# MaxChen228/pingpong-selfplay-ai

Measured on AMD Instinct MI355X. Metric: env-steps/sec (whole node) at 65536 arenas, 1/2/4/8 GPUs; CPU-ref baseline, higher is better.
Workload: dtype f64 env state / f32 QNet; 1 GPU; configs[2]: 65536 arenas/GPU, full DQN train_iterative loop (act both players + env tick + PER push/sample + double-DQN update + Adam + target sync); arenas_per_gpu=65536, global_arenas=65536, pool=8, batch=256, updates_per_vector_step=1, memory_size=1000000, parallelism=dp1 (arena shards, 1 all-reduce/update)

## Files before the change

### pingpong-selfplay-ai_amd/csrc/pm_dev.h

```cpp
#pragma once
#include <hip/hip_runtime.h>
#include <stdint.h>

#include "pongmi.h"

#ifdef PM_DIAG
static __device__ unsigned long long pm_diag_buf[256];
#define PM_STAMP(slot)                                                                 \
    do {                                                                               \
        if (threadIdx.x == 0 && blockIdx.x == 0) pm_diag_buf[(slot)] = __builtin_amdgcn_s_memrealtime(); \
    } while (0)
#define PM_STAMP_ANY(slot)                                                             \
    do {                                                                               \
        if (threadIdx.x == 0) pm_diag_buf[(slot)] = __builtin_amdgcn_s_memrealtime();  \
    } while (0)
static __device__ unsigned long long pm_diag_blk[8][4096];
#define PM_BLK_END()                                                                              \
    do {                                                                                          \
        __syncthreads();                                                                          \
        PM_BLK(2);                                                                                \
        if (threadIdx.x == 0 && blockIdx.x < 4096)                                                \
            pm_diag_blk[3][blockIdx.x] =                                                          \
                (unsigned long long)__smid() | ((unsigned long long)(__builtin_amdgcn_s_getreg(20 | (3 << 11)) & 15) << 16); \
    } while (0)
// ... 106 lines not shown
};

__device__ __forceinline__ U4 philox(uint32_t c0, uint32_t c1, uint32_t c2, uint32_t c3, uint64_t key) {
    uint32_t k0 = (uint32_t)key, k1 = (uint32_t)(key >> 32);
#pragma unroll
    for (int r = 0; r < 10; ++r) {
        const uint64_t p0 = (uint64_t)c0 * 0xD2511F53u, p1 = (uint64_t)c2 * 0xCD9E8D57u;
        const uint32_t hi0 = (uint32_t)(p0 >> 32), lo0 = (uint32_t)p0;
        const uint32_t hi1 = (uint32_t)(p1 >> 32), lo1 = (uint32_t)p1;
        const uint32_t n0 = hi1 ^ c1 ^ k0, n2 = hi0 ^ c3 ^ k1;
        c0 = n0; c1 = lo1; c2 = n2; c3 = lo0;
        k0 += 0x9E3779B9u; k1 += 0xBB67AE85u;
    }
    return {c0, c1, c2, c3};
}

__device__ __forceinline__ U4 philox64(uint32_t index, uint32_t tag, uint64_t ctr, uint64_t key) {
    return philox(index, tag, (uint32_t)ctr, (uint32_t)(ctr >> 32), key);
}

__device__ __forceinline__ double u53(uint32_t hi, uint32_t lo) {
    const uint64_t v = (((uint64_t)hi << 32) | lo) >> 11;
    return (double)v * 0x1.0p-53;
}
__device__ __forceinline__ int32_t below(uint32_t r, uint32_t n) {
    return (int32_t)(((uint64_t)r * n) >> 32);
}
__device__ __forceinline__ double det_ln_u1(uint32_t k) {
    int e = 31 - __builtin_clz(k);
    double m = (double)k / (double)(1u << e);
    if (m > 1.4142135623730951) { m = m * 0.5; e = e + 1; }
    const double s = (m - 1.0) / (m + 1.0), s2 = s * s;
    const double p = s2 * (0.66666666666666663 + s2 * (0.40000000000000002 + s2 * (0.28571428571428570 +
                     s2 * (0.22222222222222221 + s2 * (0.18181818181818182 + s2 * (0.15384615384615385 +
                     s2 * (0.13333333333333333 + s2 * (0.11764705882352941 + s2 * (0.10526315789473684 +
                     s2 * 0.09523809523809523)))))))));
    return (double)(e - 24) * 0.69314718055994531 + (2.0 * s + s * p);
}
__device__ __forceinline__ double det_cos_turn(double t) {
    const double q = floor(4.0 * t + 0.5);
    const double th = 6.2831853071795862 * (t - 0.25 * q);
    const double z = th * th;
    const double c = 1.0 + z * (-0.5 + z * (0.041666666666666664 + z * (-0.0013888888888888889 +
                     z * (2.4801587301587302e-05 + z * (-2.755731922398589e-07 + z * (2.0876756987868100e-09 +
                     z * -1.1470745597729725e-11))))));
    const double s = th * (1.0 + z * (-0.16666666666666666 + z * (0.0083333333333333332 + z * (-0.00019841269841269841 +
                     z * (2.7557319223985893e-06 + z * (-2.5052108385441720e-08 + z * (1.6059043836821613e-10 +
                     z * -7.6471637318198164e-13)))))));
    const int qi = (int)q & 3;
    return qi == 0 ? c : (qi == 1 ? -s : (qi == 2 ? -c : s));
}
__device__ __forceinline__ float normal(uint32_t a, uint32_t b) {
    const double r = sqrt(-2.0 * det_ln_u1((a >> 8) + 1u));
    return (float)(r * det_cos_turn((double)(b >> 8) * 0x1.0p-24));
}
__device__ __forceinline__ float scale_noise(float x) {
    const float s = x > 0.f ? 1.f : (x < 0.f ? -1.f : 0.f);
    return s * (float)sqrt((double)fabsf(x));
}

struct Arena {
    double x, y, vx, vy, spin, top, bot;
    int32_t sA, sB, bounces;
};

__device__ __forceinline__ Arena load_arena(const pm_env_state& s, int i) {
    Arena a;
    a.x = s.x[i]; a.y = s.y[i]; a.vx = s.vx[i]; a.vy = s.vy[i];
    a.spin = s.spin[i]; a.top = s.top[i]; a.bot = s.bot[i];
    a.sA = s.scoreA[i]; a.sB = s.scoreB[i]; a.bounces = s.bounces[i];
    return a;
}

template <bool WT, typename T>
__device__ __forceinline__ void st_out(T* p, T v) {
    if constexpr (WT) __hip_atomic_store(p, v, __ATOMIC_RELAXED, __HIP_MEMORY_SCOPE_AGENT);
    else *p = v;
}
typedef float pm_f4v __attribute__((ext_vector_type(4)));
template <bool WT>
__device__ __forceinline__ void st_f4(float4* p, float4 v) {
    if constexpr (WT) {
        const pm_f4v x = {v.x, v.y, v.z, v.w};
        asm volatile("global_store_dwordx4 %0, %1, off sc1" ::"v"(p), "v"(x) : "memory");
    } else {
        *p = v;
    }
}

template <bool WT = false>
__device__ __forceinline__ void store_arena(const pm_env_state& s, int i, const Arena& a) {
    st_out<WT>(&s.x[i], a.x); st_out<WT>(&s.y[i], a.y); st_out<WT>(&s.vx[i], a.vx); st_out<WT>(&s.vy[i], a.vy);
    st_out<WT>(&s.spin[i], a.spin); st_out<WT>(&s.top[i], a.top); st_out<WT>(&s.bot[i], a.bot);
    st_out<WT>(&s.scoreA[i], a.sA); st_out<WT>(&s.scoreB[i], a.sB); st_out<WT>(&s.bounces[i], a.bounces);
}

__device__ __forceinline__ void observe(const Arena& a, float* oA, float* oB) {
    oA[0] = (float)a.x; oA[1] = (float)(1.0 - a.y); oA[2] = (float)a.vx; oA[3] = (float)(-a.vy);
    oA[4] = (float)a.top; oA[5] = (float)a.bot; oA[6] = (float)a.spin;
    oB[0] = (float)a.x; oB[1] = (float)a.y; oB[2] = (float)a.vx; oB[3] = (float)a.vy;
    oB[4] = (float)a.bot; oB[5] = (float)a.top; oB[6] = (float)a.spin;
}

constexpr int kRowBlock = 256;

template <bool WT = false>
__device__ __forceinline__ void copy_rows7(float* __restrict__ dst, const float (*lds)[7], int i0, int n) {
    const int t = threadIdx.x;
    const int rows = min(kRowBlock, n - i0);
    float* base = dst + (size_t)i0 * 7;
    const float* src = &lds[0][0];
    if (rows == kRowBlock && (((uintptr_t)base) & 15) == 0) {
        float4* d4 = reinterpret_cast<float4*>(base);
        const float4* s4 = reinterpret_cast<const float4*>(__builtin_assume_aligned(src, 16));
#pragma unroll
        for (int f = t; f < kRowBlock * 7 / 4; f += kRowBlock) st_f4<WT>(d4 + f, s4[f]);
    } else {
        for (int f = t; f < rows * 7; f += kRowBlock) base[f] = src[f];
    }
}

__device__ __forceinline__ void store_rows7(float* __restrict__ dst, float (*lds)[7], const float* row, int i0,
                                            int n) {
    const int t = threadIdx.x;
#pragma unroll
    for (int k = 0; k < 7; ++k) lds[t][k] = row[k];
    __syncthreads();
    copy_rows7(dst, lds, i0, n);
    __syncthreads();
}

typedef float pm_f4u __attribute__((ext_vector_type(4), aligned(4)));
typedef float pm_f3u __attribute__((ext_vector_type(3), aligned(4)));
__device__ __forceinline__ void store_row7(float* __restrict__ dst, const float* v) {
    *reinterpret_cast<pm_f4u*>(dst) = pm_f4u{v[0], v[1], v[2], v[3]};
    *reinterpret_cast<pm_f3u*>(dst + 4) = pm_f3u{v[4], v[5], v[6]};
}

__device__ __forceinline__ void serve(Arena& a, double vx, double vy, double spin) {
    a.sA = 0; a.sB = 0; a.bounces = 0;
    a.top = 0.5; a.bot = 0.5; a.x = 0.5; a.y = 0.5;
    a.vx = vx; a.vy = vy; a.spin = spin;
}

__device__ __forceinline__ void sincos_serve(double x, double& s, double& c) {
    const double pio4 = 7.85398163397448278999e-01;
    const double pio2_1 = 1.57079632673412561417e+00, pio2_1t = 6.07710050650619224932e-11;
    const int n = x > pio4 ? 1 : (x < -pio4 ? -1 : 0);
    const double z0 = n > 0 ? x - pio2_1 : x + pio2_1;
    const double t = n > 0 ? pio2_1t : -pio2_1t;
    double y0 = z0 - t;
    double y1 = (z0 - y0) - t;
    y0 = n == 0 ? x : y0;
    y1 = n == 0 ? 0.0 : y1;
    const double S1 = -1.66666666666666324348e-01, S2 = 8.33333333332248946124e-03,
                 S3 = -1.98412698298579493134e-04, S4 = 2.75573137070700676789e-06,
                 S5 = -2.50507602534068634195e-08, S6 = 1.58969099521155010221e-10;
    const double z = y0 * y0, v = z * y0;
    const double rs = S2 + z * (S3 + z * (S4 + z * (S5 + z * S6)));
    const double ks = y0 - ((z * (0.5 * y1 - v * rs) - y1) - v * S1);
    const double C1 = 4.16666666666666019037e-02, C2 = -1.38888888888741095749e-03,
                 C3 = 2.48015872894767294178e-05, C4 = -2.75573143513906633035e-07,
                 C5 = 2.08757232129817482790e-09, C6 = -1.13596475577881948265e-11;
    const double rc = z * (C1 + z * (C2 + z * (C3 + z * (C4 + z * (C5 + z * C6)))));
    const double hz = 0.5 * z, w = 1.0 - hz;
    const double kc = w + (((1.0 - w) - hz) + (z * rc - y0 * y1));
    s = n == 0 ? ks : (n > 0 ? kc : -kc);
    c = n == 0 ? kc : (n > 0 ? -ks : ks);
}
// ... 168 lines not shown
```

### pingpong-selfplay-ai_amd/csrc/pm_per.h

```cpp
#pragma once
#include <hip/hip_runtime.h>
#include <stdint.h>

#include "pongmi.h"
#include "pm_dev.h"

namespace pm {

constexpr int PER_SUB = 64;
constexpr int PER_FAN = 16;
constexpr int PER_CHUNK = PER_SUB * PER_FAN;

__host__ __device__ inline int64_t per_pad(int64_t n_doubles) { return ((n_doubles * 8 + 255) / 256) * 256; }

struct PerTree {
    double* chunk;
    double* sub;
    float* leaf;
    int64_t nchunk, nsub;
};

__host__ __device__ inline PerTree per_tree(void* work, int64_t cap) {
    PerTree t;
    t.nsub = (cap + PER_SUB - 1) / PER_SUB;
    t.nchunk = (cap + PER_CHUNK - 1) / PER_CHUNK;
    char* w = reinterpret_cast<char*>(work);
    t.chunk = reinterpret_cast<double*>(w);
    t.sub = reinterpret_cast<double*>(w + per_pad(t.nchunk));
    t.leaf = reinterpret_cast<float*>(w + per_pad(t.nchunk) + per_pad(t.nsub));
    return t;
}

inline int64_t per_work_bytes(int64_t cap) {
    return per_pad((cap + PER_CHUNK - 1) / PER_CHUNK) + per_pad((cap + PER_SUB - 1) / PER_SUB) +
           ((cap * 4 + 255) / 256) * 256;
}

struct PushRange {
    int64_t pos, n, cap;
    float pval;
    __device__ __forceinline__ int64_t dist(int64_t e) const {
        const int64_t d = e - pos;
        return d < 0 ? d + cap : d;
    }
    __device__ __forceinline__ bool covers(int64_t e) const { return dist(e) < n; }
};

__device__ __forceinline__ double wave_incl_scan(double v, int lane) {
#pragma unroll
    for (int o = 1; o < 64; o <<= 1) {
        const double u = __shfl_up(v, o);
        if (lane >= o) v += u;
    }
    return v;
}

struct RingNodes {
    int64_t a0, na, nb;
    __device__ __forceinline__ int64_t count() const { return na + nb; }
    __device__ __forceinline__ int64_t at(int64_t k) const { return k < na ? a0 + k : k - na; }
};
__device__ __forceinline__ RingNodes ring_nodes(const PushRange& pr, int64_t g) {
    RingNodes r{pr.pos / g, 0, 0};
    if (pr.n <= 0) return r;
    const int64_t end1 = pr.pos + pr.n < pr.cap ? pr.pos + pr.n : pr.cap;
    r.na = (end1 - 1) / g - r.a0 + 1;
    const int64_t end2 = pr.pos + pr.n - pr.cap;
    r.nb = end2 > 0 ? (end2 - 1) / g + 1 : 0;
    return r;
}

__device__ __forceinline__ float prio_pow(float p, float alpha) {
    if (!(p > 0.f)) return 0.f;
    int e;
    double m = 2.0 * frexp((double)p, &e);
    e = e - 1;
    if (m > 1.4142135623730951) { m = m * 0.5; e = e + 1; }
    const double s = (m - 1.0) / (m + 1.0), s2 = s * s;
    const double q = s2 * (0.66666666666666663 + s2 * (0.40000000000000002 + s2 * (0.28571428571428570 +
                     s2 * (0.22222222222222221 + s2 * (0.18181818181818182 + s2 * (0.15384615384615385 +
                     s2 * (0.13333333333333333 + s2 * (0.11764705882352941 + s2 * (0.10526315789473684 +
                     s2 * 0.09523809523809523)))))))));
    const double y = (double)alpha * ((double)e * 0.69314718055994531 + (2.0 * s + s * q));
    const double k = floor(y * 1.4426950408889634 + 0.5);
    const double r = (y - k * 6.93147180369123816490e-01) - k * 1.90821492927058770002e-10;
    const double ex = 1.0 + r * (1.0 + r * (0.5 + r * (0.16666666666666666 + r * (0.041666666666666664 +
                      r * (0.008333333333333333 + r * (0.001388888888888889 + r * (0.0001984126984126984 +
                      r * (2.48015873015873e-05 + r * (2.7557319223985893e-06 + r * (2.755731922398589e-07 +
                      r * (2.505210838544172e-08 + r * (2.08767569878681e-09 + r * 1.6059043836821613e-10))))))))))));
    return (float)ldexp(ex, (int)k);
}

__device__ __forceinline__ float per_leaf(const float* __restrict__ leaf, int64_t e, const PushRange& pr) {
    return pr.covers(e) ? pr.pval : (e < pr.cap ? leaf[e] : 0.f);
}

__device__ __forceinline__ double per_quarter(const float* __restrict__ leaf, int64_t sb, int k, const PushRange pr) {
    const int64_t lo = sb * PER_SUB + 16 * k;
    float v[16];
    if (lo + 16 <= pr.cap) {
        const float4* p4 = reinterpret_cast<const float4*>(leaf + lo);
#pragma unroll
        for (int q = 0; q < 4; ++q) {
            const float4 x = p4[q];
            v[4 * q] = x.x; v[4 * q + 1] = x.y; v[4 * q + 2] = x.z; v[4 * q + 3] = x.w;
        }
    } else {
#pragma unroll
        for (int i = 0; i < 16; ++i) v[i] = lo + i < pr.cap ? leaf[lo + i] : 0.f;
    }
    const int64_t d0 = pr.dist(lo);
    double acc = 0.0;
#pragma unroll
    for (int i = 0; i < 16; ++i) {
        int64_t d = d0 + i;
        if (d >= pr.cap) d -= pr.cap;
        acc += lo + i < pr.cap ? (double)(d < pr.n ? pr.pval : v[i]) : 0.0;
    }
    return acc;
}
__device__ __forceinline__ double per_combine(double q0, double q1, double q2, double q3) {
    return ((q0 + q1) + q2) + q3;
}
__device__ __forceinline__ double per_sub_sum(const float* __restrict__ leaf, int64_t sb, const PushRange pr) {
    const double q0 = per_quarter(leaf, sb, 0, pr), q1 = per_quarter(leaf, sb, 1, pr);
    const double q2 = per_quarter(leaf, sb, 2, pr), q3 = per_quarter(leaf, sb, 3, pr);
    return per_combine(q0, q1, q2, q3);
}
__device__ __forceinline__ double per_sub_sum4(const float* __restrict__ leaf, int64_t sb, const PushRange pr) {
    const int lane = threadIdx.x & 63;
    const double q = per_quarter(leaf, sb, lane & 3, pr);
    return per_combine(quad_f64<0>(q), quad_f64<1>(q), quad_f64<2>(q), quad_f64<3>(q));
}

__device__ __forceinline__ bool per_sub_pushed(int64_t sb, const PushRange pr) {
    const int64_t lo = sb * PER_SUB;
    return lo + PER_SUB <= pr.cap && pr.dist(lo) + PER_SUB <= pr.n;
}
__device__ __forceinline__ double per_sub_pushed_sum(const PushRange pr) {
    double q = 0.0;
#pragma unroll
    for (int i = 0; i < 16; ++i) q += (double)pr.pval;
    return per_combine(q, q, q, q);
}

__device__ __forceinline__ double per_chunk_sum(const PerTree& t, int64_t c) {
    double v[PER_FAN];
#pragma unroll
    for (int k = 0; k < PER_FAN; ++k) v[k] = c * PER_FAN + k < t.nsub ? t.sub[c * PER_FAN + k] : 0.0;
    double acc = 0.0;
#pragma unroll
    for (int k = 0; k < PER_FAN; ++k) acc += v[k];
    return acc;
}

constexpr int PER_BS = 64;
constexpr int PER_ROUND = 1024;

struct PerSampleSmem {
    double incl[PER_ROUND];
    double wsum[4];
};

__device__ inline double per_round_prefix(const double (&v)[4], double base, PerSampleSmem& sm) {
    const int t = threadIdx.x, lane = t & 63, wv = t >> 6;
    double run[4], acc = 0.0;
#pragma unroll
    for (int e = 0; e < 4; ++e) { acc += v[e]; run[e] = acc; }
    const double incl = wave_incl_scan(acc, lane);
    double excl = __shfl_up(incl, 1);
    if (lane == 0) excl = 0.0;
    if (lane == 63) sm.wsum[wv] = incl;
    __syncthreads();
    double wb = base;
    for (int w = 0; w < wv; ++w) wb += sm.wsum[w];
    const double ex = wb + excl;
#pragma unroll
    for (int e = 0; e < 4; ++e) sm.incl[4 * t + e] = ex + run[e];
    const double tot = ((base + sm.wsum[0]) + sm.wsum[1]) + sm.wsum[2] + sm.wsum[3];
    __syncthreads();
    return tot;
}

__device__ __forceinline__ int per_lds_search(const PerSampleSmem& sm, int n, double x) {
    int lo = 0, hi = n;
    while (lo < hi) {
        const int mid = (lo + hi) >> 1;
        if (sm.incl[mid] > x) hi = mid;
        else lo = mid + 1;
    }
    return lo;
}

template <int NV>
__device__ __forceinline__ int per_group_find(const double (&v)[NV], double x, double& before, double& val) {
    const int lane = threadIdx.x & 63, q = lane & 3, g0 = lane & ~3;
    double acc = 0.0;
#pragma unroll
    for (int e = 0; e < NV; ++e) acc += v[e];
    const double s0 = quad_f64<0>(acc), s1 = quad_f64<1>(acc), s2 = quad_f64<2>(acc);
    const double ex = q == 0 ? 0.0 : (q == 1 ? s0 : (q == 2 ? s0 + s1 : (s0 + s1) + s2));
    double pre[NV + 1];
    pre[0] = ex;
#pragma unroll
    for (int e = 0; e < NV; ++e) pre[e + 1] = pre[e] + v[e];
    int k = -1;
    double hb = 0.0, hv = 0.0;
#pragma unroll
    for (int e = NV - 1; e >= 0; --e) {
        const bool h = pre[e + 1] > x;
        k = h ? e : k;
        hb = h ? pre[e] : hb;
        hv = h ? v[e] : hv;
    }
    const unsigned gh = (unsigned)(__ballot(k >= 0) >> g0) & 15u;
    int src;
    if (gh) {
        src = __ffs(gh) - 1;
    } else {
        hb = ex;
        hv = 0.0;
#pragma unroll
        for (int e = 0; e < NV; ++e) {
            const bool z = v[e] > 0.0;
            k = z ? e : k;
            hb = z ? pre[e] : hb;
            hv = z ? v[e] : hv;
        }
        const unsigned gn = (unsigned)(__ballot(k >= 0) >> g0) & 15u;
        src = gn ? 31 - __clz(gn) : 0;
        k = k < 0 ? 0 : k;
    }
    const int kk = quad_sel_i32(k, src);
    before = quad_sel_f64(hb, src);
    val = quad_sel_f64(hv, src);
    return src * NV + kk;
}

struct NoHook {
    __device__ void operator()() const {}
};
__device__ __forceinline__ float per_is_weight(int64_t size, double pa, double total, double beta) {
    return (float)pow((double)size * (pa / total), -beta);
}
template <bool RAW = false, class UFn, class OutFn, class Hook = NoHook>
__device__ inline void per_sample_block(bool active, int64_t size, const PerTree& tr, const PushRange& pr, double beta,
                                        int j0, int bs, PerSampleSmem& sm, UFn ufn, OutFn out, Hook l2done = Hook()) {
    const int t = threadIdx.x, q = t & 3;
    const int j = j0 + (t >> 2);
    const bool one_round = tr.nchunk <= PER_ROUND;
    double vc[4] = {0.0, 0.0, 0.0, 0.0};
    if (one_round) {
#pragma unroll
        for (int e = 0; e < 4; ++e) {
            const int64_t c = 4 * t + e;
            vc[e] = c < tr.nchunk ? tr.chunk[c] : 0.0;
        }
        asm volatile("" ::"v"(vc[0]), "v"(vc[1]), "v"(vc[2]), "v"(vc[3]));
    }
    if (!active) return;
    const int64_t nb = (size + PER_CHUNK - 1) / PER_CHUNK;
    const double u = j < bs ? ufn(j) : 0.0;
    double total = 0.0;
    if (nb > PER_ROUND) {
        for (int64_t c0 = 0; c0 < nb; c0 += PER_ROUND) {
            double v[4];
#pragma unroll
            for (int e = 0; e < 4; ++e) {
                const int64_t c = c0 + 4 * t + e;
                v[e] = c < nb ? tr.chunk[c] : 0.0;
            }
            total = per_round_prefix(v, total, sm);
        }
    }
// ... 87 lines not shown
```

### pingpong-selfplay-ai_amd/csrc/pm_selfplay.hip

```cpp
#include <algorithm>
#include <cmath>

#include "pm_host.h"
#include "pm_mfma.h"
#include "pm_per.h"

using namespace pm;

#ifdef PM_DIAG
static __device__ unsigned long long pm_diag_env[8][1024];
static __device__ unsigned long long pm_diag_side[4][1024];
#define PM_SIDE(k, sb, v)                                                        \
    do {                                                                         \
        if (threadIdx.x == 0 && (sb) < 1024) pm_diag_side[(k)][(sb)] = (v);      \
    } while (0)
#define PM_STAMP_MAX_NB(slot)                                                                              \
    do {                                                                                                   \
        if (threadIdx.x == 0) atomicMax(&pm_diag_buf[(slot)], (unsigned long long)__builtin_amdgcn_s_memrealtime()); \
    } while (0)
#define PM_ENV_STAMP(k, blk)                                                                   \
    do {                                                                                       \
        asm volatile("" ::: "memory");                                                         \
        if (threadIdx.x == 0 && (blk) < 1024) pm_diag_env[(k)][(blk)] = __builtin_amdgcn_s_memrealtime(); \
    } while (0)
#define PM_ENV_STAMP_DRAIN(k, blk)                                                             \
    do {                                                                                       \
        asm volatile("s_waitcnt vmcnt(0) lgkmcnt(0)" ::: "memory");                            \
        if (threadIdx.x == 0 && (blk) < 1024) pm_diag_env[(k)][(blk)] = __builtin_amdgcn_s_memrealtime(); \
    } while (0)
#else
#define PM_SIDE(k, sb, v) \
    do {                  \
    } while (0)
#define PM_STAMP_MAX_NB(slot) \
    do {                      \
    } while (0)
#define PM_ENV_STAMP(k, blk) \
    do {                     \
    } while (0)
#define PM_ENV_STAMP_DRAIN(k, blk) \
    do {                           \
    } while (0)
#endif

namespace {

constexpr int kBlock = 256;
static_assert(kBlock == kRowBlock, "row staging assumes kRowBlock-thread blocks");
constexpr int kLearn = 1024;
constexpr int kGradN = PM_GRAD_EPISODES;
static_assert(PM_GRAD_EPISODES == PM_QNET_NHEAD && PM_GRAD_UPDATED == kGradN + 1 && PM_GRAD_LEN >= kGradN + 2, "grad layout");
constexpr uint32_t kHashEmpty = 0xFFFFFFFFu;

__device__ __forceinline__ bool learner_active(const pm_selfplay& sp) {
    const int64_t s = sp.ctrl->size + sp.n;
    return (s < sp.cap ? s : sp.cap) >= sp.batch;
}

__device__ __forceinline__ double beta_of(const pm_selfplay& sp, int64_t frame) {
    const double b = sp.beta_start + (double)frame * (1.0 - sp.beta_start) / (double)sp.beta_frames;
    return b < 1.0 ? b : 1.0;
}

__device__ __forceinline__ float push_prio(int64_t size, float max_prio) { return size == 0 ? 1.0f : max_prio; }
__device__ __forceinline__ PushRange push_of(const pm_selfplay& sp, int64_t pos, int64_t size, float max_prio) {
    return PushRange{pos, sp.n, sp.cap, prio_pow(push_prio(size, max_prio), (float)sp.alpha)};
}
}

__device__ __forceinline__ void sample_block(const pm_selfplay& sp, int b, bool pending, PerSampleSmem& sm) {
    const pm_ctrl* c = sp.ctrl;
    const int64_t s = c->size + sp.n;
    const int64_t size = s < sp.cap ? s : sp.cap;
    const int64_t frame = c->frame_idx + 1;
    const PushRange pr = pending ? push_of(sp, c->pos, c->size, c->max_prio) : PushRange{0, 0, sp.cap, 0.f};
    const uint64_t key = sp.seed_env;
    per_sample_block(
        size >= sp.batch, size, per_tree(sp.per_work, sp.cap), pr, beta_of(sp, frame), b * PER_BS,
        min(sp.batch, b * PER_BS + PER_BS), sm,
        [&](int j) {
            const U4 r = philox64((uint32_t)j, TAG_PER, (uint64_t)frame, key);
            return u53(r.x, r.y);
        },
        [&](int j, int64_t idx, float w) {
            sp.idx[j] = idx;
            sp.isw[j] = w;
        });
}

union ActSpShared {
    ActShared act;
    PerSampleSmem per;
};
constexpr int kFeatTilesAct = 8, kFeatTilesLearn = 16;
#ifndef PM_ENV_WT
#define PM_ENV_WT 6
#endif
constexpr bool kEnvWTRows = (PM_ENV_WT & 1) != 0, kEnvWTState = (PM_ENV_WT & 2) != 0, kEnvWTObs = (PM_ENV_WT & 4) != 0;
__host__ __device__ inline int feat_ntiles(int n) { return (n + 31) / 32; }

__device__ __forceinline__ bool gb_current(const pm_selfplay& sp) {
    return sp.featB && sp.gB && sp.gB_ready && !sp.frow;
}
__device__ __forceinline__ uint32_t* gh_epoch(const pm_selfplay& sp) {
    return reinterpret_cast<uint32_t*>(sp.gheads + PM_GHEADS_EPOCH);
}
constexpr int kAheadPollMax = 20000;
__device__ __forceinline__ void gh_publish(const pm_selfplay& sp, int k, uint32_t tag, float v) {
    __hip_atomic_store(sp.gheads + k, ((uint64_t)tag << 32) | __float_as_uint(v), __ATOMIC_RELAXED, __HIP_MEMORY_SCOPE_AGENT);
}

struct FeatAheadSmem {
    float lw[kLwFloats];
    float hf[264];
    int ok;
};
__device__ __forceinline__ void feat_tiles_ahead(const pm_selfplay& sp, FeatAheadSmem& sm, int t0, int t1, bool force_timeout) {
    const int t = threadIdx.x, wave = t >> 6, lane = t & 63, nw = blockDim.x >> 6;
    stage_frags_lds(sp.w_B, sm.lw, t0);
    const uint32_t tag = __hip_atomic_load(gh_epoch(sp), __ATOMIC_RELAXED, __HIP_MEMORY_SCOPE_AGENT) + 1u;
    const int tl[2] = {t0 + wave, t0 + wave + nw};
    const bool has[2] = {tl[0] < t1, tl[1] < t1};
    float xs[2][4] = {{0.f, 0.f, 0.f, 0.f}, {0.f, 0.f, 0.f, 0.f}};
#pragma unroll
    for (int k = 0; k < 2; ++k)
        if (has[k]) tile_inputs(sp.obsB + (size_t)min(tl[k] * 32 + (lane & 31), sp.n - 1) * 7, lane >> 5, xs[k]);
    if (t == 0) sm.ok = 1;
    __syncthreads();
    f32x16 c2[2][2] = {};
#pragma unroll
    for (int k = 0; k < 2; ++k)
        if (has[k]) tile_hidden(sm.lw, xs[k], lane, c2[k]);
    PM_STAMP_MAX_NB(68);
    if (t < 260) {
        const int c = t & 3, r = (t >> 2) & 15, tt = (t >> 6) & 1, h = t >> 7;
        const int src = t < 256 ? c * 64 + 32 * tt + rho(r) + 4 * h : t;
        uint64_t g = 0;
        bool got = false;
        for (int it = 0; !force_timeout && it < kAheadPollMax; ++it) {
            g = __hip_atomic_load(sp.gheads + src, __ATOMIC_RELAXED, __HIP_MEMORY_SCOPE_AGENT);
            if ((uint32_t)(g >> 32) == tag) { got = true; break; }
            __builtin_amdgcn_s_sleep(2);
        }
        if (got) sm.hf[t] = __uint_as_float((uint32_t)g);
        else sm.ok = 0;
    }
    __syncthreads();
    PM_STAMP_MAX_NB(69);
    const bool ok = sm.ok != 0;
#pragma unroll
    for (int k = 0; k < 2; ++k) {
        if (!has[k]) continue;
        const int arena = tl[k] * 32 + (lane & 31);
        int a = PM_GB_NONE;
        if (ok) {
            float q[3];
            tile_heads(sm.hf, c2[k], lane, q);
            a = argmax3(q);
        } else {
            feat_store(sp.featB, tl[k], lane, c2[k]);
        }
        if (lane < 32 && arena < sp.n) sp.gB[arena] = (int8_t)a;
    }
}

__global__ __launch_bounds__(kActBlock, 4) void k_act_sp(const pm_selfplay sp, int part) {
    __shared__ __attribute__((aligned(16))) ActSpShared sh;
    PM_BLK(0);
    const int nsb = part == PM_ACT_A ? 0 : (sp.batch + PER_BS - 1) / PER_BS;
    {
        const ActGrid g{sp.n, sp.n_pool + 1, sp.chunk_A, sp.chunk_P, part == PM_ACT_A ? 0 : 1};
        const int fb = (int)blockIdx.x - nsb - g.blocks();
        if (fb >= 0) {
            const int t0 = fb * kFeatTilesAct;
            feat_tiles(sh.act.lw, sp.w_B, sp.obsB, sp.n, t0, min(t0 + kFeatTilesAct, feat_ntiles(sp.n)), sp.featB);
            return;
        }
    }
    if ((int)blockIdx.x < nsb) {
        PM_STAMP(64);
        sample_block(sp, (int)blockIdx.x, true, sh.per);
// ... 144 lines not shown
        w2r[2 * m] = odd ? f2[m].y : f2[m].x;
        w2r[2 * m + 1] = odd ? f2[m].w : f2[m].z;
    }
    {
        const float x0 = g == 0 ? 1.0f : o0;
        const f32x4v16 zero = {0.f, 0.f, 0.f, 0.f};
        f32x4v16 c1 = __builtin_amdgcn_mfma_f32_16x16x4f32(w1r[0], x0, zero, 0, 0, 0);
        c1 = __builtin_amdgcn_mfma_f32_16x16x4f32(w1r[1], x1, c1, 0, 0, 0);
#pragma unroll
        for (int r = 0; r < 4; ++r) {
            const int q = l2_pos(16 * rt + 4 * g + r), sq = q >> 2;
            sm.h1s[q & 3][sq >> 2][col][sq & 3] = relu(c1[r]);
        }
    }
    __syncthreads();
    float hw4[32];
    {
        const float* src = sm.opw[lane >> 5][(lane >> 4) & 1][lane & 3];
#pragma unroll
        for (int k = 0; k < 8; ++k) {
            const float4 w = *reinterpret_cast<const float4*>(src + 4 * k);
            hw4[4 * k] = w.x; hw4[4 * k + 1] = w.y; hw4[4 * k + 2] = w.z; hw4[4 * k + 3] = w.w;
        }
    }
    const float4 bhr = *reinterpret_cast<const float4*>(sm.hf + (lane >> 5) * 264 + 256);
    float bs[16];
#pragma unroll
    for (int k = 0; k < 4; ++k) {
        const float4 v = *reinterpret_cast<const float4*>(sm.h1s[g][k][col]);
        bs[4 * k] = v.x; bs[4 * k + 1] = v.y; bs[4 * k + 2] = v.z; bs[4 * k + 3] = v.w;
    }
    f32x4v16 c2 = {b2r.x, b2r.y, b2r.z, b2r.w};
#pragma unroll
    for (int i = 0; i < 16; ++i) c2 = __builtin_amdgcn_mfma_f32_16x16x4f32(w2r[i], bs[i], c2, 0, 0, 0);
    float* row = sp.hfeat + (size_t)j * 80;
#pragma unroll
    for (int r = 0; r < 4; ++r) {
        const int u = 16 * rt + 4 * g + r, q = head_pos(u);
        c2[r] = relu(c2[r]);
        sm.c2s[(u >> 2) & 1][q >> 2][col][q & 3] = c2[r];
    }
    if (mine && !nxt) *reinterpret_cast<float4*>(row + 16 * rt + 4 * g) = make_float4(c2[0], c2[1], c2[2], c2[3]);
    __syncthreads();
    if (rt != 0) return;
    if (wj >= 0) sp.isw[wj] = wisw;
    const int set = lane >> 5, hh = (lane >> 4) & 1;
    float xb[32];
#pragma unroll
    for (int k = 0; k < 8; ++k) {
        const float4 x = *reinterpret_cast<const float4*>(sm.c2s[hh][k][col]);
        xb[4 * k] = x.x; xb[4 * k + 1] = x.y; xb[4 * k + 2] = x.z; xb[4 * k + 3] = x.w;
    }
    f32x4v16 acc = {0.f, 0.f, 0.f, 0.f};
#pragma unroll
    for (int q = 0; q < 32; ++q) acc = __builtin_amdgcn_mfma_f32_4x4x1f32(hw4[q], xb[q], acc, 0, 0, 0);
    float v = xor16_sum(acc[0]), a0 = xor16_sum(acc[1]), a1 = xor16_sum(acc[2]), a2 = xor16_sum(acc[3]);
    v += bhr.x;
    a0 += bhr.y;
    a1 += bhr.z;
    a2 += bhr.w;
    const float mean = ((a0 + a1) + a2) / 3.0f;
    const float q0 = v + (a0 - mean), q1 = v + (a1 - mean), q2 = v + (a2 - mean);
    if (mine && hh == 0) {
        if (set == 0) {
            float* qd = row + (nxt ? 68 : 64);
            qd[0] = q0; qd[1] = q1; qd[2] = q2;
            if (!nxt) {
                row[67] = rb0;
                row[71] = rb1;
            }
        } else if (nxt) {
            row[72] = q0; row[73] = q1; row[74] = q2;
        }
    }
}

__device__ __forceinline__ void write_opp_lists(const pm_selfplay& sp, OppListSmem& sm, int blk, int i, bool valid,
                                                int net) {
    write_opp_lists(sp.n_pool + 1, sp.opp_list, sp.opp_cnt, sm, blk, i, valid, net);
}

struct EnvSmem {
    float lds[2][kBlock][7];
    long long red[kBlock / 64][6];
    OppListSmem ol;
};
struct ActEnvSmem {
    EnvSmem e;
    float lw[kLwFloats];
};

template <bool ACT>
__device__ __forceinline__ void env_block(const pm_selfplay& sp, int blk, EnvSmem& sm, float* lw) {
    const int i0 = blk * kBlock;
    const int i = i0 + threadIdx.x;
    const int lane = threadIdx.x & 63, wv = threadIdx.x >> 6;
    const bool valid = i < sp.n;
    const int ii = valid ? i : sp.n - 1;
    const pm_ctrl* c = sp.ctrl;
    if (blk == 0) PM_STAMP_ANY(72);
    PM_ENV_STAMP(0, blk);
    float xs[2][4];
    f32x16 fc2[2][2];
    const bool ahead = ACT && gb_current(sp);
    if (ahead) {
    } else if (ACT && sp.featB) {
        if (threadIdx.x < 65)
            reinterpret_cast<float4*>(lw + F_H)[threadIdx.x] =
                reinterpret_cast<const float4*>(sp.w_B + PLAIN + F_H)[threadIdx.x];
        const int tlast = feat_ntiles(sp.n) - 1;
#pragma unroll
        for (int k = 0; k < 2; ++k) feat_load(sp.featB, min(blk * 8 + 2 * wv + k, tlast), lane, fc2[k]);
    } else if (ACT) {
        stage_frags_lds(sp.w_B, lw, blk);
#pragma unroll
        for (int k = 0; k < 2; ++k) {
            const int row = min(i0 + 64 * wv + 32 * k + (lane & 31), sp.n - 1);
            tile_inputs(sp.obsB + (size_t)row * 7, lane >> 5, xs[k]);
        }
    }
    const uint32_t ns = (uint32_t)__builtin_nontemporal_load(&sp.st.serves[ii]);
    const int64_t pos = c->pos, size = c->size;
    const float cmaxp = c->max_prio;
    const uint64_t cstep = c->step;
    const double ceps = c->epsilon;
    const int o = sp.opp[ii];
    const float er0 = sp.ep_reward[ii];
    Arena a = load_arena(sp.st, ii);
    const int aA = sp.aA[ii];
    int aB = ACT ? (ahead ? (int)sp.gB[ii] : 0) : sp.aB[ii];
    __builtin_amdgcn_sched_barrier(0);
    const float maxp = push_prio(size, cmaxp);
    float* leaf = per_tree(sp.per_work, sp.cap).leaf;
    const float pval = prio_pow(maxp, (float)sp.alpha);

    int onext, eps_a;
    bool eps_hit;
    double svx, svy, sspn;
    {
        const U4 rr = philox64((uint32_t)ii, TAG_ACT, cstep, sp.seed_env);
        eps_hit = u53(rr.x, rr.y) < ceps;
        eps_a = (int)below(rr.z, 3u);
        const U4 q = philox((uint32_t)ii, TAG_OPP, ns, 0u, sp.seed_env);
        onext = (sp.n_pool > 0 && u53(q.x, q.y) < sp.pool_ratio) ? 1 + below(q.z, (uint32_t)sp.n_pool) : 0;
        philox_serve(sp.env, (uint32_t)ii, ns, sp.seed_env, svx, svy, sspn);
        asm volatile("" ::"v"(onext), "v"(svx), "v"(svy), "v"(sspn), "v"(eps_hit), "v"(eps_a));
        __builtin_amdgcn_sched_barrier(0);
    }
    if (ahead) {
        const unsigned long long fb = __ballot(valid && aB == PM_GB_NONE);
        if (fb) {
#pragma unroll
            for (int k = 0; k < 2; ++k) {
                if (!(uint32_t)(fb >> (32 * k))) continue;
                float q[3];
                feat_load(sp.featB, blk * 8 + 2 * wv + k, lane, fc2[k]);
                tile_heads(sp.w_B + PLAIN + F_H, fc2[k], lane, q);
                if ((lane >> 5) == k) aB = argmax3(q);
            }
        }
        if (!valid) aB = 0;
        PM_ENV_STAMP(7, blk);
    } else if (ACT) {
        __syncthreads();
        PM_ENV_STAMP(7, blk);
        int act[2];
#pragma unroll
        for (int k = 0; k < 2; ++k) {
            float q[3];
            if (sp.featB) {
                tile_heads(lw + F_H, fc2[k], lane, q);
            } else {
                f32x16 c2[2];
                tile_hidden(lw, xs[k], lane, c2);
                tile_heads(lw + F_H, c2, lane, q);
            }
            act[k] = argmax3(q);
            if (sp.featB && sp.frow) {
                const int ar = i0 + 64 * wv + 32 * k + (lane & 31);
                if (ar < sp.n) {
                    int64_t slot = pos + ar;
                    if (slot >= sp.cap) slot -= sp.cap;
                    float4* fr = reinterpret_cast<float4*>(sp.frow + slot * 64) + (lane >> 5);
#pragma unroll
                    for (int jt = 0; jt < 2; ++jt)
#pragma unroll
                        for (int q4 = 0; q4 < 4; ++q4)
                            st_f4<kEnvWTRows>(fr + 8 * jt + 2 * q4,
                                              make_float4(relu(fc2[k][jt][4 * q4]), relu(fc2[k][jt][4 * q4 + 1]),
                                                          relu(fc2[k][jt][4 * q4 + 2]), relu(fc2[k][jt][4 * q4 + 3])));
                }
            }
        }
        aB = lane < 32 ? act[0] : act[1];
    }
    PM_ENV_STAMP(1, blk);
    if (eps_hit) aB = eps_a;
    float oA[7], oB[7];
    observe(a, oA, oB);
    float rA, rB;
    const int d = tick(sp.env, a, aA, aB, rA, rB);
    float nA[7], nB[7];
    observe(a, nA, nB);
#ifdef PM_DIAG
    asm volatile("" ::"v"(nA[0]), "v"(nB[1]), "v"(d));
#endif
    PM_ENV_STAMP(2, blk);
    const float er = er0 + rB;
    const bool fin = valid && d;
    {
        const bool win = er > 0.f;
        const unsigned long long mf = __ballot(fin), mA = __ballot(fin && o == 0), mwA = __ballot(fin && o == 0 && win);
        const unsigned long long mP = __ballot(fin && o != 0), mwP = __ballot(fin && o != 0 && win);
        const int rs = wave_sum(fin ? (int)er : 0);
        if (lane == 0) {
            sm.red[wv][0] = __popcll(mf); sm.red[wv][1] = __popcll(mA); sm.red[wv][2] = __popcll(mwA);
            sm.red[wv][3] = __popcll(mP); sm.red[wv][4] = __popcll(mwP); sm.red[wv][5] = rs;
        }
    }
    int onew = o;
    if (valid) {
        int64_t slot = pos + i;
        if (slot >= sp.cap) slot -= sp.cap;
        float4* row = reinterpret_cast<float4*>(sp.trans + slot * PM_TRANS_F);
        st_f4<kEnvWTRows>(row + 0, make_float4(oB[0], oB[1], oB[2], oB[3]));
        st_f4<kEnvWTRows>(row + 1, make_float4(oB[4], oB[5], oB[6], rB));
        st_f4<kEnvWTRows>(row + 2, make_float4(nB[0], nB[1], nB[2], nB[3]));
        st_f4<kEnvWTRows>(row + 3, make_float4(nB[4], nB[5], nB[6], __int_as_float(aB | (d << 8))));
        sp.prios[slot] = maxp;
        leaf[slot] = pval;
        float ernew = er;
        if (d) {
            onew = onext;
            serve(a, svx, svy, sspn);
            sp.st.serves[i] = (int32_t)ns + 1;
            ernew = 0.f;
            observe(a, nA, nB);
        }
        store_arena<kEnvWTState>(sp.st, i, a);
        sp.opp[i] = onew;
        sp.aB[i] = (int8_t)aB;
        sp.ep_reward[i] = ernew;
    }
    PM_ENV_STAMP(3, blk);
#pragma unroll
    for (int k = 0; k < 7; ++k) { sm.lds[0][threadIdx.x][k] = nA[k]; sm.lds[1][threadIdx.x][k] = nB[k]; }
    __syncthreads();
    PM_ENV_STAMP(4, blk);
    if (threadIdx.x < 6) {
        long long t = 0;
        for (int w = 0; w < kBlock / 64; ++w) t += sm.red[w][threadIdx.x];
        sp.partials[(size_t)blk * 8 + threadIdx.x] = t;
    }
    write_opp_lists(sp, sm.ol, blk, i, valid, onew);
    PM_ENV_STAMP(5, blk);
    copy_rows7<kEnvWTObs>(sp.obsA, sm.lds[0], i0, sp.n);
    copy_rows7<kEnvWTObs>(sp.obsB, sm.lds[1], i0, sp.n);
    PM_ENV_STAMP_DRAIN(6, blk);
}

__global__ __launch_bounds__(kBlock) void k_env(const pm_selfplay sp) {
    const int blk = (int)blockIdx.x;
    const int nenv = (sp.n + kBlock - 1) / kBlock;
    if (blk >= nenv) {
        env_fwd_block(sp, blk - nenv);
        return;
    }
    __shared__ __attribute__((aligned(16))) EnvSmem sm;
    env_block<false>(sp, blk, sm, nullptr);
}

union ActEnvShared {
    ActEnvSmem ae;
    SampleFwd16Smem sf16;
};
__global__ __launch_bounds__(kBlock) void k_actenv(const pm_selfplay sp) {
    __shared__ __attribute__((aligned(16))) ActEnvShared sh;
    const int nsb = (sp.batch + kSampBlock - 1) / kSampBlock;
    if ((int)blockIdx.x < nsb) {
        PM_BLK(0);
        sample_fwd_block16(sp, (int)blockIdx.x, sh.sf16);
        PM_BLK_END();
        return;
    }
    env_block<true>(sp, (int)blockIdx.x - nsb, sh.ae.e, sh.ae.lw);
}

__global__ __launch_bounds__(kBlock) void k_sp_init(const pm_selfplay sp) {
    __shared__ __attribute__((aligned(16))) float lds[kBlock][7];
    const int i0 = blockIdx.x * kBlock;
    const int i = i0 + threadIdx.x;
    float oA[7] = {0}, oB[7] = {0};
    int net = 0;
    if (i < sp.n) {
        const uint32_t ns = (uint32_t)sp.st.serves[i];
        const U4 q = philox((uint32_t)i, TAG_OPP, ns, 0u, sp.seed_env);
        net = (sp.n_pool > 0 && u53(q.x, q.y) < sp.pool_ratio) ? 1 + below(q.z, (uint32_t)sp.n_pool) : 0;
        sp.opp[i] = net;
        Arena a;
        double vx, vy, spn;
        philox_serve(sp.env, (uint32_t)i, ns, sp.seed_env, vx, vy, spn);
        serve(a, vx, vy, spn);
        store_arena(sp.st, i, a);
        sp.st.serves[i] = (int32_t)ns + 1;
        sp.ep_reward[i] = 0.f;
        observe(a, oA, oB);
    }
    {
        __shared__ OppListSmem ol;
        write_opp_lists(sp, ol, blockIdx.x, i, i < sp.n, net);
    }
    store_rows7(sp.obsA, lds, oA, i0, sp.n);
    store_rows7(sp.obsB, lds, oB, i0, sp.n);
// ... 1926 lines not shown
```

Measured before the change: 2.186 billion env-steps/s.

## Coalesce transition-row stores via LDS staging, DPP scan, 4-ary LDS search

Transition rows are now staged through LDS per wave so each store instruction writes contiguous 64-byte rows across lanes, replacing four strided per-lane row stores. The write-through default now also covers transition rows, while feature-row and priority stores get their own write-through flags. The PER sampling wave scan is rebuilt on DPP row shifts and permlane swaps instead of shuffles, and the LDS binary search becomes a 4-ary search with parallel probes. This adds LDS footprint and wave barriers in the env kernel, and the s_nop after each write-through store adds a little issue latency.

```diff
diff --git a/pingpong-selfplay-ai_amd/csrc/pm_dev.h b/pingpong-selfplay-ai_amd/csrc/pm_dev.h
--- a/pingpong-selfplay-ai_amd/csrc/pm_dev.h
+++ b/pingpong-selfplay-ai_amd/csrc/pm_dev.h
@@ -212,9 +212,33 @@
 __device__ __forceinline__ void st_f4(float4* p, float4 v) {
     if constexpr (WT) {
         const pm_f4v x = {v.x, v.y, v.z, v.w};
-        asm volatile("global_store_dwordx4 %0, %1, off sc1" ::"v"(p), "v"(x) : "memory");
+        asm volatile("global_store_dwordx4 %0, %1, off sc1\n\ts_nop 1" ::"v"(p), "v"(x) : "memory");
     } else {
         *p = v;
+    }
+}
+
+template <bool WT>
+__device__ __forceinline__ void store_ring_rows16(float* __restrict__ ring, int64_t pos, int64_t cap, int r0, int n,
+                                                  float4 (*stage)[4], const float4 (&piece)[4]) {
+    const int lane = threadIdx.x & 63;
+#pragma unroll
+    for (int k = 0; k < 4; ++k) stage[lane][k] = piece[k];
+    __builtin_amdgcn_fence(__ATOMIC_RELEASE, "wavefront");
+    __builtin_amdgcn_wave_barrier();
+    __builtin_amdgcn_fence(__ATOMIC_ACQUIRE, "wavefront");
+    const float4* flat = &stage[0][0];
+    float4 x[4];
+#pragma unroll
+    for (int k = 0; k < 4; ++k) x[k] = flat[lane + 64 * k];
+    asm volatile("" : "+v"(x[0].x), "+v"(x[1].x), "+v"(x[2].x), "+v"(x[3].x));
+#pragma unroll
+    for (int k = 0; k < 4; ++k) {
+        const float4 v = x[k];
+        const int row = r0 + (lane >> 2) + 16 * k;
+        int64_t slot = pos + row;
+        if (slot >= cap) slot -= cap;
+        if (row < n) st_f4<WT>(reinterpret_cast<float4*>(ring + slot * 16) + (lane & 3), v);
     }
 }
 
diff --git a/pingpong-selfplay-ai_amd/csrc/pm_per.h b/pingpong-selfplay-ai_amd/csrc/pm_per.h
--- a/pingpong-selfplay-ai_amd/csrc/pm_per.h
+++ b/pingpong-selfplay-ai_amd/csrc/pm_per.h
@@ -51,6 +51,47 @@
     for (int o = 1; o < 64; o <<= 1) {
         const double u = __shfl_up(v, o);
         if (lane >= o) v += u;
+    }
+    return v;
+}
+
+__device__ __forceinline__ double wave_shr1_f64(double v) {
+    const unsigned long long x = (unsigned long long)__double_as_longlong(v);
+    const unsigned lo = (unsigned)__builtin_amdgcn_update_dpp(0, (int)(unsigned)x, 0x138, 0xF, 0xF, true);
+    const unsigned hi = (unsigned)__builtin_amdgcn_update_dpp(0, (int)(unsigned)(x >> 32), 0x138, 0xF, 0xF, true);
+    return __longlong_as_double((long long)(((unsigned long long)hi << 32) | lo));
+}
+__device__ __forceinline__ double wave_incl_scan_dpp(double v, int lane) {
+#pragma unroll
+    for (int o = 1; o < 16; o <<= 1) {
+        double u = v;
+#pragma unroll
+        for (int s = 0; s < o; ++s) u = wave_shr1_f64(u);
+        v += u;
+    }
+    const int row = lane >> 4;
+    {
+        const unsigned long long x = (unsigned long long)__double_as_longlong(v);
+        unsigned w[2];
+#pragma unroll
+        for (int h = 0; h < 2; ++h) {
+            const unsigned d = (unsigned)(x >> (32 * h));
+            const auto p = __builtin_amdgcn_permlane16_swap(d, d, false, false);
+            const auto m = __builtin_amdgcn_permlane32_swap(p[1], p[1], false, false);
+            w[h] = row == 0 ? 0u : (row == 2 ? m[0] : p[0]);
+        }
+        v += __longlong_as_double((long long)(((unsigned long long)w[1] << 32) | w[0]));
+    }
+    {
+        const unsigned long long x = (unsigned long long)__double_as_longlong(v);
+        unsigned w[2];
+#pragma unroll
+        for (int h = 0; h < 2; ++h) {
+            const unsigned d = (unsigned)(x >> (32 * h));
+            const auto p = __builtin_amdgcn_permlane32_swap(d, d, false, false);
+            w[h] = row < 2 ? 0u : p[0];
+        }
+        v += __longlong_as_double((long long)(((unsigned long long)w[1] << 32) | w[0]));
     }
     return v;
 }
@@ -167,9 +208,8 @@
     double run[4], acc = 0.0;
 #pragma unroll
     for (int e = 0; e < 4; ++e) { acc += v[e]; run[e] = acc; }
-    const double incl = wave_incl_scan(acc, lane);
-    double excl = __shfl_up(incl, 1);
-    if (lane == 0) excl = 0.0;
+    const double incl = wave_incl_scan_dpp(acc, lane);
+    const double excl = wave_shr1_f64(incl);
     if (lane == 63) sm.wsum[wv] = incl;
     __syncthreads();
     double wb = base;
@@ -183,13 +223,20 @@
 }
 
 __device__ __forceinline__ int per_lds_search(const PerSampleSmem& sm, int n, double x) {
-    int lo = 0, hi = n;
-    while (lo < hi) {
-        const int mid = (lo + hi) >> 1;
-        if (sm.incl[mid] > x) hi = mid;
-        else lo = mid + 1;
-    }
-    return lo;
+    static_assert(PER_ROUND == 1024, "per_lds_search's five base-4 digits");
+    int base = 0;
+#pragma unroll
+    for (int stride = 256; stride >= 1; stride >>= 2) {
+        const int np = stride == 256 ? 4 : 3;
+        double v[4];
+#pragma unroll
+        for (int i = 0; i < np; ++i) v[i] = sm.incl[min(base + stride * (i + 1) - 1, n - 1)];
+        int cnt = 0;
+#pragma unroll
+        for (int i = 0; i < np; ++i) cnt += (base + stride * (i + 1) - 1 < n && !(v[i] > x)) ? 1 : 0;
+        base += stride * cnt;
+    }
+    return base;
 }
 
 template <int NV>
diff --git a/pingpong-selfplay-ai_amd/csrc/pm_selfplay.hip b/pingpong-selfplay-ai_amd/csrc/pm_selfplay.hip
--- a/pingpong-selfplay-ai_amd/csrc/pm_selfplay.hip
+++ b/pingpong-selfplay-ai_amd/csrc/pm_selfplay.hip
@@ -94,9 +94,11 @@
 };
 constexpr int kFeatTilesAct = 8, kFeatTilesLearn = 16;
 #ifndef PM_ENV_WT
-#define PM_ENV_WT 6
+#define PM_ENV_WT 7
 #endif
 constexpr bool kEnvWTRows = (PM_ENV_WT & 1) != 0, kEnvWTState = (PM_ENV_WT & 2) != 0, kEnvWTObs = (PM_ENV_WT & 4) != 0;
+constexpr bool kEnvWTPrio = (PM_ENV_WT & 8) != 0;
+constexpr bool kEnvWTFrow = (PM_ENV_WT & 16) != 0;
 __host__ __device__ inline int feat_ntiles(int n) { return (n + 31) / 32; }
 
 __device__ __forceinline__ bool gb_current(const pm_selfplay& sp) {
@@ -407,6 +409,7 @@
 
 struct EnvSmem {
     float lds[2][kBlock][7];
+    float4 rows[kBlock][4];
     long long red[kBlock / 64][6];
     OppListSmem ol;
 };
@@ -511,7 +514,7 @@
                     for (int jt = 0; jt < 2; ++jt)
 #pragma unroll
                         for (int q4 = 0; q4 < 4; ++q4)
-                            st_f4<kEnvWTRows>(fr + 8 * jt + 2 * q4,
+                            st_f4<kEnvWTFrow>(fr + 8 * jt + 2 * q4,
                                               make_float4(relu(fc2[k][jt][4 * q4]), relu(fc2[k][jt][4 * q4 + 1]),
                                                           relu(fc2[k][jt][4 * q4 + 2]), relu(fc2[k][jt][4 * q4 + 3])));
                 }
@@ -544,16 +547,18 @@
         }
     }
     int onew = o;
+    {
+        static_assert(PM_TRANS_F == 16, "store_ring_rows16 writes 64-byte rows");
+        const float4 piece[4] = {make_float4(oB[0], oB[1], oB[2], oB[3]), make_float4(oB[4], oB[5], oB[6], rB),
+                                 make_float4(nB[0], nB[1], nB[2], nB[3]),
+                                 make_float4(nB[4], nB[5], nB[6], __int_as_float(aB | (d << 8)))};
+        store_ring_rows16<kEnvWTRows>(sp.trans, pos, sp.cap, i0 + 64 * wv, sp.n, sm.rows + 64 * wv, piece);
+    }
     if (valid) {
         int64_t slot = pos + i;
         if (slot >= sp.cap) slot -= sp.cap;
-        float4* row = reinterpret_cast<float4*>(sp.trans + slot * PM_TRANS_F);
-        st_f4<kEnvWTRows>(row + 0, make_float4(oB[0], oB[1], oB[2], oB[3]));
-        st_f4<kEnvWTRows>(row + 1, make_float4(oB[4], oB[5], oB[6], rB));
-        st_f4<kEnvWTRows>(row + 2, make_float4(nB[0], nB[1], nB[2], nB[3]));
-        st_f4<kEnvWTRows>(row + 3, make_float4(nB[4], nB[5], nB[6], __int_as_float(aB | (d << 8))));
-        sp.prios[slot] = maxp;
-        leaf[slot] = pval;
+        st_out<kEnvWTPrio>(&sp.prios[slot], maxp);
+        st_out<kEnvWTPrio>(&leaf[slot], pval);
         float ernew = er;
         if (d) {
             onew = onext;
```

New measurement: 2.330 billion env-steps/s, median of 6. 1.07x the previous value.
